# dvrp0/Monsoon

Hardware: AMD Instinct MI355X
Metric: env-steps/sec (whole node) at 65536 concurrent games; bit-exact vs CPU replay (higher is better)
Workload: dtype u8/i16 state, f64 draw+score

## Files before the change

monsoon_amd/csrc/abilities.inc:

```

MSB_HD MSB_INL PList sel_targets(int shape, P c, int pov, Tgt t) { return shape_targets(shape, c, pov, t, PK_NONE); }

MSB_HD MSB_INL bool sel_any(int shape, P c, int pov, Tgt t) { return shape_any(shape, c, pov, t); }

MSB_HD MSB_A_TILES PList empty_shape_tiles(int shape, P c, int pov) {
  PList raw = shape_tiles(shape, c, pov);
  PList out;
  out.clear();
  int m = raw.n();
  for (int i = 0; i < m; i++)
    if (at(raw.at(i)) == AT_NONE) out.push_raw(raw.get(i));
  return out;
}
MSB_HD MSB_A_TILES PList empty_within_front_line(int order) {
  PList out;
  out.clear();
  int fl = pl_front(order);
  if (order == 0) {
    for (int y = fl; y < 5; y++)
      for (int x = 0; x < 4; x++) {
        P p{x, y};
        if (at(p) == AT_NONE) out.push(p);
      }
  } else {
// ... 106 lines not shown
      const int who = at(l.at(i));
      if (who < 0 || who >= AT_PLAYER) {
        set_fault(who < 0 ? FAULT_PY_EXCEPTION : FAULT_UNSUPPORTED);
        break;
      }
      const int s = e_str(who);
      const int dealt = s - 3 < 0 ? s : 3;
      if (dealt < -128) set_fault(FAULT_UNSUPPORTED);
      cur = dealt & 0xff;
      call_damage(k, who, 3, true);
    } break;
    case EACH_DMG_RAND: {
      const int t = at(l.at(i));
      if (t < 0) {
        set_fault(FAULT_PY_EXCEPTION);
        break;
      }
      const int dmg = rng_randint(4, 6);
      call_damage(k, t, dmg, true);
    } break;
    case EACH_DESTROY: {
      const int t = at(l.at(i));
      if (t < 0 || t >= AT_PLAYER) {
        set_fault(t < 0 ? FAULT_PY_EXCEPTION : FAULT_UNSUPPORTED);
        break;
      }
      call_destroy(k, t, true);
    } break;
    case EACH_COMMAND:
      call_command(k, at(l.at(i)));
      break;
    case EACH_COMMAND_B203: {
      const int t = at(l.at(i));
      if (!need_unit(t)) break;
      if (e_confused(t)) deconfuse(t);
      if (fault()) break;
      call_command(k, t);
    } break;
    case EACH_U018: {
      Tgt t = mk_tgt(TK_ANY, TS_ENEMY);
      t = tgt_base(t);
      const PList l2 = get_targets(cp(), t, PK_NONE);
      call_damage(k, at(choice_point(l2)), 2, true);
    } break;
    case EACH_UE01: {
      const PList l2 = get_targets(arg, mk_tgt(TK_UNIT, TS_ENEMY), PK_NONE);
      if (l2.n() > 0) call_damage(k, at(choice_point(l2)), 1, true);
      else skip = true;
    } break;
    case EACH_U017: {
      const int me = cur;
      const int oi = l.get(i);
      int idx = oi;
      for (int q = 0; q < oi; q++)
        if (arg & (1 << q)) idx--;
      const CardInfo& ci = g_cards[hand_card(me, idx)];
      P pos{0, 0};
      bool has_pos = false;
      if (ci.tgt.has) {
        const PList l2 = get_targets(cp(), mk_tgt(ci.tgt), PK_NONE);
        if (l2.n() == 0) {
          set_fault(FAULT_PY_EXCEPTION);
          break;
        }
        pos = choice_point(l2);
        has_pos = true;
      }
      arg |= 1 << oi;
      call_player_play(k, me, idx, pos, has_pos);
    } break;
    default:
      set_fault(FAULT_UNSUPPORTED);
      break;
  }
  if (fault()) return;
  if (skip) {
    if (counts) n--;
    else i++;
  }
  m.sk_st(top - 1, (uint32_t)op | ((uint32_t)(arg & 0xff) << 8) | (counts ? (uint32_t)(n & 0xffff) << 16 : ((uint32_t)(i & 0xff) << 16) | ((uint32_t)(n & 0xff) << 24)));
  m.sk_st(top, mk_hdr(F_EACH, skip ? 0 : 1, e, cur));
}

enum : int {
  AFTER_U076 = 1,
  AFTER_U302,
  AFTER_B305,
};
MSB_HD MSB_INL void call_after(Wk& k, int op, int e, int t, int aux) {
  wk_push(k, (uint32_t)aux);
  wk_push(k, mk_hdr(F_AFTER, op, e, t));
}
MSB_HD MSB_INL void h_after(Wk& k, const uint32_t hdr) {
  const int top = k.sp - 1;
  const int op = hdr_st(hdr), t = hdr_b(hdr);
  const int aux = (int)m.sk_ld(top - 1);
  k.sp = top - 1;
  switch (op) {
// ... 34 lines not shown
    MSB_CARD_LOCALS                                                        \
    switch (0) {                                                           \
      default: __VA_ARGS__                                                 \
    }                                                                      \
  }
#define MSB_CARD_K(id, ...)                                                \
  MSB_HD MSB_A_RARE int ab_##id(int sp_, int deep_, int e, int pos_pk, bool src) { \
    Wk k{sp_, 0, deep_, 0};                                                \
    const int card = id;                                                   \
    MSB_CARD_LOCALS                                                        \
    switch (0) {                                                           \
      default: __VA_ARGS__                                                 \
    }                                                                      \
    return k.sp;                                                           \
  }
#define MSB_SPELL(id, ...)                                                 \
  MSB_HD MSB_A_CARD void sp_##id(int me, int pos_pk) {                     \
    const int card = id;                                                   \
    MSB_SPELL_LOCALS                                                       \
    switch (0) {                                                           \
      default: __VA_ARGS__                                                 \
    }                                                                      \
  }
#define MSB_SPELL_K(id, ...)                                               \
  MSB_HD MSB_A_RARE int sp_##id(int sp_, int deep_, int me, int pos_pk) {  \
    Wk k{sp_, 0, deep_, 0};                                                \
    const int card = id;                                                   \
    MSB_SPELL_LOCALS                                                       \
    switch (0) {                                                           \
      default: __VA_ARGS__                                                 \
    }                                                                      \
    return k.sp;                                                           \
  }
#include "ability_cases.inc"
#undef MSB_CARD
#undef MSB_CARD_K
#undef MSB_SPELL
#undef MSB_SPELL_K

MSB_HD MSB_INL void ability_entity_card(Wk& k, int card, int e, int pos_pk, bool src) {
  switch (card) {
#define MSB_CARD(id, ...) case id: ab_##id(e, pos_pk, src); break;
#define MSB_CARD_K(id, ...) case id: k.sp = ab_##id(k.sp, k.base - k.seg, e, pos_pk, src); break;
#define MSB_SPELL(id, ...)
#define MSB_SPELL_K(id, ...)
#include "ability_cases.inc"
#undef MSB_CARD
#undef MSB_CARD_K
#undef MSB_SPELL
#undef MSB_SPELL_K
    default:
      if (card_has_ability(card)) set_fault(FAULT_UNSUPPORTED);
      break;
  }
}
MSB_HD MSB_INL void ability_entity(Wk& k, int e, int pos_pk, bool src) {
  MSB_SCOPE(PS_ABILITY_ENTITY);
  const int card = e_card(e);
#if defined(__HIP_DEVICE_COMPILE__)
  int cv = card;
  asm volatile("" : "+v"(cv));
  for (unsigned long long todo = __ballot(1); todo;) {
    const int leader = __builtin_ctzll(todo);
    const int c0 = __builtin_amdgcn_readlane(card, leader), c1 = __builtin_amdgcn_readlane(cv, leader);
    const bool mine = card == c0;
    todo &= ~__ballot(mine);
    if (mine) {
// ... 47 lines not shown
```

monsoon_amd/csrc/ability_cases.inc:

```

MSB_CARD_K(C_B002, {
      l = get_targets(dpov, mk_tgt(TK_ANY, TS_ENEMY), PK_NONE);
      if (l.n() > 0) {
        l = sorted_head(l, 0, true, 1);
        call_damage(k, at(l.at(0)), 8, true);
      }
    } break;
)
MSB_CARD_K(C_B004, {
      Tgt t = mk_tgt(TK_ANY, TS_ENEMY);
      t = tgt_base(t);
      l = get_targets(dpov, t, PK_NONE);
      call_each(k, EACH_DMG_B004, e, l, l.n(), 4, 0);
    } break;
)
MSB_CARD(C_B005, {
      if (!REM_LISTS) {
        set_fault(FAULT_UNSUPPORTED);
        break;
      }
      l = sel_targets(SH_SURROUNDING, mypos, dpov, mk_tgt(TK_ANY, TS_FRIENDLY));
      int mine = m.ld8(E_REM + e);
      if (mine == REM_LOST) {
        set_fault(FAULT_CAP_REM);
// ... 125 lines not shown
      if (l.n() > 0) {
        l = sorted_head(l, 1, false, 1);
        call_destroy(k, at(l.at(0)), true);
      }
    } break;
)
MSB_CARD(C_B009, {
      l = get_targets(dpov, mk_tgt(TK_UNIT, TS_ENEMY), PK_NONE);
      if (l.n() > 0) {
        l = sorted_head(l, 0, true, 2);
        l = shuffle(l);
        for (int i = 0; i < l.n() && !fault(); i++) confuse(at(l.at(i)));
      }
    } break;
)
MSB_CARD(C_B104, {
      l = get_targets(dpov, mk_tgt(TK_UNIT, TS_ENEMY), PK_NONE);
      if (l.n() > 0) {
        l = sorted_head(l, 0, true, 1);
        freeze(at(l.at(0)));
      }
    } break;
)
MSB_CARD_K(C_B203, {
      l = sel_targets(SH_FRONT, mypos, me, mk_tgt(TK_UNIT, TS_FRIENDLY));
      call_each(k, EACH_COMMAND_B203, e, l, l.n(), 0, 0);
    } break;
)
MSB_CARD_K(C_B304,
      call_entity_damage(k, e, 3, false, true);
      break;
)
MSB_CARD(C_U007, {
      l = sel_targets(SH_SURROUNDING, mypos, me, mk_tgt(TK_UNIT, TS_ENEMY));
      if (l.n() > 0) {
        int t = at(choice_point(l));
        heal(t, 5);
        vitalize(t);
      }
    } break;
)
MSB_CARD_K(C_U017, {
      int hn = pl_hand_n(me);
      PList orig;
      orig.clear();
      for (int i = 0; i < hn; i++) {
        int c = hand_card(me, i);
        if (c < NUM_CARDS && g_cards[c].kind == KIND_SPELL && hand_cost(me, i) <= 8) orig.push_raw(i);
      }
      int nc = orig.n();
      if (nc == 0) break;
      orig = shuffle(orig);
      int remaining = 8;
      PList pick;
      pick.clear();
      for (int i = 0; i < nc; i++) {
        int cost = hand_cost(me, orig.get(i));
        if (cost <= remaining) {
          pick.push_raw(orig.get(i));
          remaining -= cost;
        }
      }
      call_each(k, EACH_U017, e, pick, pick.n(), 0, me);
    } break;
)
MSB_CARD_K(C_U018, {
      l = sel_targets(SH_SURROUNDING, mypos, dpov, mk_tgt(TK_UNIT, TS_ANY));
      int types = 0, cnt = 0;
      for (int i = 0; i < l.n(); i++) {
        int b = 1 << card_first_type(e_card(at(l.at(i))));
        if (!(types & b)) {
          types |= b;
          cnt++;
        }
      }
      call_each(k, EACH_U018, e, l, cnt, 0, 0);
    } break;
)
MSB_CARD(C_U021, {
      l = get_targets(dpov, mk_tgt(TK_UNIT, TS_FRIENDLY), p_pack(mypos));
      if (l.n() > 0) heal(at(choice_point(l)), 5);
    } break;
)
MSB_CARD_K(C_U026, {
      l = sel_targets(SH_BEHIND, mypos, dpov, mk_tgt(TK_ANY, TS_ENEMY));
      if (l.n() > 0) call_damage(k, at(l.at(0)), 6, true);
    } break;
)
MSB_CARD(C_U036,
      if (pl_hand_n(me) == 0) heal(at(mypos), 12);
      break;
)
MSB_CARD(C_U040, {
      if (src) {
        l = shape_tiles(SH_SURROUNDING, mypos, me);
        if (l.n() > 0) respawn(e, choice_point(l), 12);
      }
    } break;
)
MSB_CARD(C_U050,
      if (mypos.y == 4) gain_speed(e, 3);
      break;
)
MSB_CARD(C_U051, {
      if (!sel_any(SH_BORDERING, mypos, dpov, mk_tgt(TK_UNIT, TS_ANY)))
        gain_speed(e, 1);
      else
        heal(e, 2);
    } break;
)
MSB_CARD(C_U053, {
      if (!sel_any(SH_SURROUNDING, mypos, dpov, mk_tgt(TK_UNIT, TS_ANY))) {
        gain_speed(e, 2);
      } else {
        if (!sel_any(SH_BORDERING, mypos, dpov, mk_tgt(TK_UNIT, TS_ANY))) gain_speed(e, 1);
      }
    } break;
)
MSB_CARD(C_U055, {
      Tgt t = mk_tgt(TK_UNIT, TS_ENEMY);
      t = tgt_xstatus(t, 1 << ST_CONFUSED);
      l = sel_targets(SH_FRONT, mypos, dpov, t);
      for (int i = 0; i < l.n() && !fault(); i++) confuse(at(l.at(i)));
    } break;
)
MSB_CARD(C_U061, {
      confuse(e);
      l = get_targets(dpov, mk_tgt(TK_UNIT, TS_FRIENDLY), p_pack(mypos));
      if (l.n() > 0) confuse(at(choice_point(l)));
      gain_speed(e, 2);
    } break;
)
MSB_CARD(C_U071, {
      l = sel_targets(SH_BORDERING, mypos, me, mk_tgt(TK_UNIT, TS_ENEMY));
      PList nc;
      nc.clear();
      for (int i = 0; i < l.n(); i++)
        if (!e_confused(at(l.at(i)))) nc.push_raw(l.get(i));
      if (nc.n() > 0) {
        confuse(at(choice_point(nc)));
        l = shape_tiles(SH_FRONT, mypos, dpov);
        if (l.n() > 0 && at(l.at(0)) == AT_NONE) teleport(e, l.at(0));
      }
    } break;
)
MSB_CARD_K(C_U074, {
      l = sel_targets(SH_FRONT, mypos, me, mk_tgt(TK_UNIT, TS_ENEMY));
      if (l.n() > 0) call_force_attack(k, e, l.at(0));
    } break;
)
MSB_CARD_K(C_U076, {
      Tgt t = mk_tgt(TK_UNIT, TS_ANY);
      t = tgt_xtypes(t, 1 << UT_DRAGON);
      l = sel_targets(SH_SURROUNDING, mypos, dpov, t);
      if (l.n() > 0) {
        int target = at(choice_point(l));
        call_after(k, AFTER_U076, e, target, me);
        call_damage(k, target, 6, true);
      }
    } break;
)
MSB_CARD_K(C_U101, {
      P position = p_unpack(pos_pk);
      int t = at(position);
      if (p_is_base(position) || t < 0 || t >= AT_PLAYER || !e_is_unit(t) || !e_frozen(t)) break;
      Tgt tg = mk_tgt(TK_UNIT, TS_ENEMY);
      tg = tgt_status(tg, 1 << ST_FROZEN);
      l = sel_targets(SH_SURROUNDING, mypos, me, tg);
      call_each(k, EACH_DMG, e, l, l.n(), 8, 0);
    } break;
)
MSB_CARD(C_U103, {
      l = sel_targets(SH_BORDERING, mypos, dpov, mk_tgt(TK_UNIT, TS_ENEMY));
      for (int i = 0; i < l.n() && !fault(); i++) freeze(at(l.at(i)));
    } break;
)
MSB_CARD(C_U106, {
      if (sel_any(SH_BORDERING, mypos, dpov, mk_tgt(TK_STRUCTURE, TS_FRIENDLY)) || mypos.y == 4) heal(e, 7);
    } break;
)
MSB_CARD(C_U111, {
      for (int k = 0; k < 10 && !fault(); k++) {
        l = sel_targets(SH_SURROUNDING, mypos, me, mk_tgt(TK_UNIT, TS_FRIENDLY));
        if (l.n() > 0) heal(at(choice_point(l)), 1);
      }
    } break;
)
MSB_CARD(C_U117,
      freeze(e);
      break;
)
MSB_CARD(C_U206,
      player_deal_damage(me, 3);
      break;
)
MSB_CARD(C_U211, {
      l = shape_tiles(SH_FRONT, mypos, dpov);
      if (l.n() > 0 && at(l.at(0)) == AT_NONE) {
        int s = rng_randint(1, 3);
        spawn_token_unit(me, l.at(0), s, UT_SATYR);
      }
    } break;
)
MSB_CARD(C_U216,
      player_deal_damage(me, 2);
      break;
)
MSB_CARD(C_U217, {
      l = empty_shape_tiles(SH_ROW, P{0, 4}, dpov);
      if (l.n() > 0) spawn_token_unit(me, choice_point(l), 5, UT_SATYR);
    } break;
)
MSB_CARD_K(C_U302, {
      P position = p_unpack(pos_pk);
      int t = at(position);
      if (p_is_base(position) || t < 0 || t >= AT_PLAYER || !e_is_unit(t)) break;
      if (e_str(t) > e_str(e)) {
        call_after(k, AFTER_U302, e, t, p_tile(mypos));
        call_entity_damage(k, t, 7, false, true);
      }
    } break;
)
MSB_CARD(C_U305, {
      Tgt t = mk_tgt(TK_UNIT, TS_FRIENDLY);
      t = tgt_types(t, 1 << UT_CONSTRUCT);
      l = sel_targets(SH_BORDERING, mypos, dpov, t);
      if (l.n() > 0) {
        heal(at(choice_point(l)), 4);
        heal(e, 4);
      }
    } break;
)
MSB_CARD_K(C_U306, {
      l = get_targets(dpov, mk_tgt(TK_ANY, TS_FRIENDLY), p_pack(mypos));
      if (l.n() > 0) call_damage(k, at(choice_point(l)), 1, true);
    } break;
)
MSB_CARD(C_U310, {
      l = sel_targets(SH_BORDERING, mypos, dpov, mk_tgt(TK_UNIT, TS_ENEMY));
      int behind = -1, right = -1, left = -1, front = -1;
      for (int i = 0; i < l.n(); i++) {
        P t = l.at(i);
        if (behind < 0 && mypos.y + 1 == t.y) behind = i;
        if (right < 0 && mypos.x + 1 == t.x) right = i;
        if (left < 0 && mypos.x - 1 == t.x) left = i;
        if (front < 0 && mypos.y - 1 == t.y) front = i;
      }
      int target = -1;
      if (behind >= 0 && l.at(behind).y < 4 && at(P{l.at(behind).x, l.at(behind).y + 1}) == AT_NONE)
        target = behind;
      else if (left >= 0 && l.at(left).x > 0 && at(P{l.at(left).x - 1, l.at(left).y}) == AT_NONE)
        target = left;
      else if (right >= 0 && l.at(right).x < 3 && at(P{l.at(right).x + 1, l.at(right).y}) == AT_NONE)
        target = right;
      else if (front >= 0 && l.at(front).y > 0 && at(P{l.at(front).x, l.at(front).y - 1}) == AT_NONE)
        target = front;
      if (target < 0) {
        set_fault(FAULT_PY_EXCEPTION);
        break;
      }
      push_pull(at(l.at(target)), mypos, true);
    } break;
)
MSB_CARD(C_U313, {
      l = sel_targets(SH_SURROUNDING, mypos, dpov, mk_tgt(TK_UNIT, TS_FRIENDLY));
      if (l.n() > 0) heal(at(choice_point(l)), 5);
      heal(e, 5);
    } break;
)
MSB_CARD(C_U314, {
      l = sel_targets(SH_FRONT, mypos, dpov, mk_tgt(TK_UNIT, TS_FRIENDLY));
      if (l.n() > 0) push_pull(at(l.at(0)), mypos, true);
    } break;
)
MSB_CARD(C_U316, {
      l = sel_targets(SH_SURROUNDING, mypos, dpov, mk_tgt(TK_UNIT, TS_FRIENDLY));
      if (l.n() > 0) {
        l = shuffle(l);
        for (int i = 0; i < l.n() && i < 2 && !fault(); i++) vitalize(at(l.at(i)));
      }
      vitalize(e);
    } break;
)
MSB_CARD(C_U320, {
      l = sel_targets(SH_SURROUNDING, mypos, me, mk_tgt(TK_UNIT, TS_FRIENDLY));
      if (l.n() > 0) heal(at(choice_point(l)), 4);
    } break;
)
MSB_CARD_K(C_U401, {
      l = sel_targets(SH_BORDERING, mypos, dpov, mk_tgt(TK_UNIT, TS_ANY));
      call_each(k, EACH_DMG_POISON, e, l, l.n(), 5, 0);
    } break;
)
MSB_CARD(C_U403, {
      Tgt t = mk_tgt(TK_UNIT, TS_ANY);
      t = tgt_status(t, 1 << ST_POISONED);
      l = sel_targets(SH_SURROUNDING, mypos, dpov, t);
      for (int i = 0; i < l.n() && !fault(); i++) {
        PList tiles;
        tiles = empty_shape_tiles(SH_BORDERING, l.at(i), dpov);
        tiles = shuffle(tiles);
        for (int k = 0; k < tiles.n() && k < 4 && !fault(); k++) spawn_token_unit(me, tiles.at(k), 1, UT_TOAD);
      }
    } break;
)
MSB_CARD_K(C_U405, {
      l = sel_targets(SH_BORDERING, mypos, dpov, mk_tgt(TK_UNIT, TS_ANY));
      call_each(k, EACH_DMG_HEAL, e, l, l.n(), 3, 0);
    } break;
)
MSB_CARD(C_U406, {
      l = empty_shape_tiles(SH_BORDERING, mypos, dpov);
      if (l.n() > 0) {
        P tile = choice_point(l);
        spawn_token_unit(opponent_of(me), tile, 1, UT_RAVEN);
      }
    } break;
)
MSB_CARD(C_U411, {
// ... 24 lines not shown
        l.clear();
        for (int i = 0; i < side.n(); i++)
          if (e_str(at(side.at(i))) == mn) l.push_raw(side.get(i));
        if (l.n() > 0) call_destroy(k, at(choice_point(l)), true);
      }
    } break;
)
MSB_CARD(C_UA05, {
      l = empty_shape_tiles(SH_SIDE, mypos, dpov);
      for (int i = 0; i < l.n() && !fault(); i++) spawn_token_unit(me, l.at(i), 4, UT_ANCIENT);
    } break;
)
MSB_CARD(C_UA07, {
      switch (rng_randint(0, 5)) {
        case 0: freeze(e); break;
        case 1: poison(e); break;
        case 2: vitalize(e); break;
        case 3: confuse(e); break;
        case 4: disable(e); break;
      }
    } break;
)
MSB_CARD(C_UA20, {
      if (!sel_any(SH_FRONT, mypos, me, mk_tgt(TK_UNIT, TS_ENEMY))) {
        const int cand[4] = {C_B005, C_B006, C_B203, C_B305};
        int c = cand[rng_randint(0, 4)];
        if (ctx() == 0) push_new_instance(me, false, c, 0, CF_SINGLE_USE | CF_XBASE, g_cards[c].strength);
      }
    } break;
)
MSB_CARD(C_UD01, {
      Tgt t = mk_tgt(TK_UNIT, TS_FRIENDLY);
      t = tgt_types(t, 1 << UT_DRAGON);
      l = get_targets(me, t, PK_NONE);
      if (l.n() > 0) heal(at(choice_point(l)), 7);
    } break;
)
MSB_CARD_K(C_UD02, {
      Tgt t = mk_tgt(TK_UNIT, TS_ANY);
      t = tgt_xtypes(t, 1 << UT_DRAGON);
      l = sel_targets(SH_FRONT, mypos, dpov, t);
      call_each(k, EACH_DMG, e, l, l.n(), 4, 0);
    } break;
)
MSB_CARD(C_UD31, {
      P position = p_unpack(pos_pk);
      int t = at(position);
      if (p_is_base(position) || t < 0 || t >= AT_PLAYER || !e_is_unit(t)) break;
      Tgt tg = mk_tgt(TK_UNIT, TS_FRIENDLY);
      tg = tgt_types(tg, 1 << UT_DRAGON);
      l = sel_targets(SH_SURROUNDING, mypos, me, tg);
      if (l.n() > 0) heal(at(choice_point(l)), 2);
      heal(e, 2);
    } break;
)
MSB_CARD_K(C_UE01, {
      int n = e_dmg(e);
      if (n > 0xffff) set_fault(FAULT_UNSUPPORTED);
      l.clear();
      if (n > 0 && n <= 0xffff) call_each(k, EACH_UE01, e, l, n, me, 0);
    } break;
)
MSB_CARD(C_UE03, {
      l = empty_shape_tiles(SH_BORDERING, mypos, dpov);
      if (l.n() > 0) {
        P tile = choice_point(l);
        spawn_token_unit(me, tile, e_str(e), UT_ELDER);
      }
    } break;
)
MSB_CARD(C_UE04, {
      l = get_targets(me, mk_tgt(TK_UNIT, TS_ENEMY), PK_NONE);
      int cnt = 0;
      for (int i = 0; i < l.n(); i++)
        if (e_str(at(l.at(i))) > e_str(e)) cnt++;
      heal(e, cnt * 4);
    } break;
)
MSB_CARD(C_UE05, {
      Tgt t = mk_tgt(TK_UNIT, TS_FRIENDLY);
      t = tgt_limit(t, e_str(e) - 1);
      l = get_targets(me, t, p_pack(mypos));
      for (int i = 0; i < l.n() && i < 4; i++) e_set_str(at(l.at(i)), e_str(e));
    } break;
)
// ... 54 lines not shown
MSB_CARD(C_UP03, {
      l = get_targets(dpov, mk_tgt(TK_UNIT, TS_FRIENDLY), PK_NONE);
      int types = 0;
      for (int i = 0; i < l.n(); i++) types |= card_types(e_card(at(l.at(i))));
      int amount = 3 * __builtin_popcount(types);
      l = sel_targets(SH_SURROUNDING, mypos, dpov, mk_tgt(TK_UNIT, TS_ENEMY));
      for (int i = 0; i < l.n(); i++) {
        int t = at(l.at(i));
        int s = e_str(t) - amount;
        e_set_str(t, s > 1 ? s : 1);
      }
    } break;
)

MSB_SPELL_K(C_S001,
      call_damage(k, at(position), 9, true);
      break;
)
MSB_SPELL_K(C_S003, {
      l = get_targets(dpov, mk_tgt(TK_ANY, TS_ENEMY), PK_NONE);
      call_each(k, EACH_DMG_RAND, 0xff, l, l.n(), 0, 0);
    } break;
)
MSB_SPELL(C_S004, {
      l = empty_within_front_line(me);
      if (l.n() > 0) {
        l = shuffle(l);
        int amount = rng_randint(6, 7);
        for (int i = 0; i < l.n() && i < amount && !fault(); i++) spawn_token_unit(me, l.at(i), 1, UT_TOAD);
      }
    } break;
)
MSB_SPELL(C_S007, {
      int t = at(position);
      heal(t, 7);
      if (!fault()) vitalize(t);
    } break;
)
MSB_SPELL(C_S012, {
      l = empty_within_front_line(me);
      if (l.n() > 0) spawn_token_unit(me, choice_point(l), 5, UT_KNIGHT);
    } break;
)
MSB_SPELL_K(C_S013, {
      PList picked;
      picked.clear();
      for (int ut = 0; ut < 16; ut++) {
        Tgt t = mk_tgt(TK_UNIT, TS_ANY);
        t = tgt_types(t, 1 << ut);
        l = get_targets(dpov, t, PK_NONE);
        PList units;
        units.clear();
        for (int i = 0; i < l.n(); i++)
          if (!picked.has(l.at(i))) units.push_raw(l.get(i));
        if (units.n() > 0) picked.push(choice_point(units));
      }
      call_each(k, EACH_DMG, 0xff, picked, picked.n(), 6, 0);
    } break;
)
MSB_SPELL(C_S021, {
      confuse(at(position));
      if (fault()) break;
      Tgt t = mk_tgt(TK_UNIT, TS_FRIENDLY);
      t = tgt_types(t, 1 << UT_FELINE);
      l = get_targets(dpov, t, PK_NONE);
      if (l.n() > 0) {
        int mn = 32767;
        for (int i = 0; i < l.n(); i++) {
          int s = e_str(at(l.at(i)));
          if (s < mn) mn = s;
        }
        PList w;
        w.clear();
        for (int i = 0; i < l.n(); i++)
// ... 14 lines not shown
    } break;
)
MSB_SPELL_K(C_S104, {
      int t = at(position);
      if (!need_unit(t)) break;
      if (e_frozen(t))
        call_entity_damage(k, t, 12, false, true);
      else
        freeze(t);
    } break;
)
MSB_SPELL(C_S105,
      heal(at(position), 15);
      break;
)
MSB_SPELL_K(C_S203, {
      l = s203_targets(dpov);
      call_each(k, EACH_DMG, 0xff, l, l.n(), 6, 0);
    } break;
)
MSB_SPELL_K(C_S302, {
      Tgt t = mk_tgt(TK_ANY, TS_ENEMY);
      t = tgt_base(t);
      l = get_targets(dpov, t, PK_NONE);
      l = shuffle(l);
      call_each(k, EACH_DMG, 0xff, l, l.n() < 4 ? l.n() : 4, 4, 0);
    } break;
)
MSB_SPELL(C_S403, {
      Tgt t = mk_tgt(TK_UNIT, TS_FRIENDLY);
      t = tgt_status(t, 1 << ST_POISONED);
      l = get_targets(dpov, t, PK_NONE);
      for (int i = 0; i < l.n() && !fault(); i++) {
        int u = at(l.at(i));
        heal(u, 5);
        if (!fault()) vitalize(u);
      }
    } break;
)
```

monsoon_amd/csrc/rules.h:

```cpp
#pragma once
#include "mt19937.h"
#include "pyset.h"
#include "state.h"

#if defined(MSB_FAULT_TRACE) && !defined(__HIPCC__)
#include <execinfo.h>
#include <stdio.h>
static inline void msb_fault_trace(int code) {
  void* bt[24];
  int n = backtrace(bt, 24);
  fprintf(stderr, "set_fault(%d)\n", code);
  backtrace_symbols_fd(bt, n, 2);
}
#endif

#if defined(MSB_COUNT_FRAMES) && !defined(__HIPCC__)
#define MSB_COUNT_EVENT(i_) msb_frame_count[i_]++
#define MSB_COUNT_MAX(i_, v_) (msb_frame_count[i_] = (v_) > msb_frame_count[i_] ? (v_) : msb_frame_count[i_])
static long long msb_frame_count[64];
#else
#define MSB_COUNT_EVENT(i_)
#define MSB_COUNT_MAX(i_, v_)
#endif

// ... 1404 lines not shown
#else
    return shape_targets_full(shape, c, pov, t, exclude_pk);
#endif
  }
  MSB_HD MSB_INL PList shape_targets_full(int shape, P c, int pov, Tgt t, int exclude_pk) {
    PList all = get_targets_full(pov, t, exclude_pk);
    PList out;
    out.clear();
    bool base_rule = shape_base_rule(shape);
    int m = all.n();
    for (int i = 0; i < m; i++) {
      P p = all.at(i);
      if (in_shape(shape, c, pov, p) || (base_rule && p_is_base(p) && tg_base(t))) out.push_raw(all.get(i));
    }
    if (shape == SH_FRONT || shape == SH_BEHIND) sort_by_y(out, (shape == SH_FRONT) ? (pov == local()) : (pov == remote()));
    return out;
  }
  MSB_HD MSB_INL bool shape_any(const int shape, const P c, const int pov, const Tgt t) {
#if MSB_TARGET_SCAN
    MSB_SCOPE(PS_GET_TARGETS);
    if (get_targets_hit(pov, t, shape_mask(shape, c, pov)) != 0) return true;
    const int bases = target_bases(t);
    if (!bases) return false;
    const bool asc = (pov == local());
    return shape_base_rule(shape) || ((bases & 1) && in_shape(shape, c, pov, base_point(true, asc))) ||
           ((bases & 2) && in_shape(shape, c, pov, base_point(false, asc)));
#else
    return shape_targets_full(shape, c, pov, t, PK_NONE).n() > 0;
#endif
  }

  MSB_HD MSB_INL int choice_index(int n) { return rng_randint(0, n); }
  MSB_HD MSB_INL P choice_point(PList l) { return l.at(choice_index(l.n())); }
  MSB_HD MSB_A_SHUFFLE PList shuffle(PList l) {
    for (int i = l.n() - 1; i >= 1; i--) {
      int j = (int)rng_interval((uint32_t)i);
      int tmp = l.get(i);
      l.set(i, l.get(j));
      l.set(j, tmp);
    }
    return l;
  }
  MSB_HD MSB_A_SHUFFLE PList sorted_head(PList l, int key_mode, bool rev, int k) {
    int b0 = -1, b1 = -1, k0 = 0, k1 = 0;
    double r0 = 0.0, r1 = 0.0;
    int m = l.n();
    for (int i = 0; i < m; i++) {
      P p = l.at(i);
      int kv = key_mode == 0 ? p.y : e_str(at(p));
      double rv = rng_random_sample();
      bool lt0 = b0 < 0 || (rev ? (kv > k0 || (kv == k0 && rv > r0)) : (kv < k0 || (kv == k0 && rv < r0)));
      if (lt0) {
        b1 = b0; k1 = k0; r1 = r0;
        b0 = i; k0 = kv; r0 = rv;
      } else {
        bool lt1 = b1 < 0 || (rev ? (kv > k1 || (kv == k1 && rv > r1)) : (kv < k1 || (kv == k1 && rv < r1)));
        if (lt1) {
          b1 = i; k1 = kv; r1 = rv;
        }
      }
    }
    PList out;
    out.clear();
    if (b0 >= 0 && k >= 1) out.push_raw(l.get(b0));
    if (b1 >= 0 && k >= 2) out.push_raw(l.get(b1));
    return out;
// ... 278 lines not shown
#else
  MSB_HD MSB_INL void call_destroy(Wk& k, int e, bool src) {
    const int sv = ctx_enter(e);
    if (fault()) return;
    wk_push_ctx(k, sv);
    if (e_is_unit(e)) {
      board_set(e_pos(e), -1);
      m.st8g(eg(e), EO_PATHN, 0);
      e_set_dmg(e, e_str(e));
      if (e_card_trigger(e) == TR_ON_DEATH) {
        push_trigger(e, src);
        if (fault()) return;
        if (!m.ld8(H_RESOLVING)) {
          wk_push(k, mk_hdr(F_DESTROY_TAIL, 0, 0, 0));
          call_pop_trigger(k);
          return;
        }
      }
      recalc_front_after_destroy();
    } else {
      e_set_dmg(e, e_str(e));
      board_set(e_pos(e), -1);
      recalc_front_after_destroy();
    }
  }
#endif
  MSB_HD MSB_INL bool need_unit(int e) {
    if (e < 0 || e >= AT_PLAYER || !e_is_unit(e)) {
      set_fault(FAULT_PY_EXCEPTION);
      return false;
    }
    return true;
  }
  MSB_HD MSB_INL void freeze(int e) {
    if (need_unit(e)) e_st_add(e, ST_FROZEN);
  }
  MSB_HD MSB_INL void poison(int e) {
    if (!need_unit(e)) return;
    if (e_st(e, ST_VITALIZED) > 0) e_st_remove(e, ST_VITALIZED);
    e_st_add(e, ST_POISONED);
  }
  MSB_HD MSB_INL void vitalize(int e) {
    if (!need_unit(e)) return;
    if (e_st(e, ST_POISONED) > 0) e_st_remove(e, ST_POISONED);
    e_st_add(e, ST_VITALIZED);
  }
  MSB_HD MSB_INL void confuse(int e) {
    if (need_unit(e)) e_st_add(e, ST_CONFUSED);
  }
  MSB_HD MSB_INL void deconfuse(int e) {
    if (need_unit(e)) e_st_remove(e, ST_CONFUSED);
  }
  MSB_HD MSB_INL void disable(int e) {
    if (need_unit(e) && e_has_ability(e)) e_st_add(e, ST_DISABLED);
  }

  MSB_HD MSB_INL void set_path(int e, bool on_play) {
    const int sv = ctx_enter(e);
    set_path_impl(e, on_play);
    ctx_leave(sv);
  }
#if MSB_WE_IMG && MSB_WIDE_PATH
  MSB_HD MSB_A_SETPATH void set_path_impl(int e, bool on_play) { set_path_known(e, on_play, m.ld32g(eg(e), 0)); }
  MSB_HD MSB_A_SETPATH void set_path_known(int e, bool on_play, const uint32_t ge) {
#else
  MSB_HD MSB_A_SETPATH void set_path_impl(int e, bool on_play) {
#endif
    MSB_SCOPE(PS_SET_PATH);
#if MSB_WIDE_PATH
    static_assert(EO_CARD == 0 && EO_FLAGS == 1 && EO_POS == 2 && EO_MOV == 3, "word 0 of an entity");
#if !MSB_WE_IMG
    const uint32_t ge = m.ld32g(eg(e), 0);
#endif
    P position = tile_p((int)(ge >> 16) & 0xff);
    int confused_cached = e_st(e, ST_CONFUSED);
    const int owner = (int)(ge >> 8) & EF_OWNER;
    const bool ff = ((ge >> 8) & EF_FF) != 0;
    const bool is_local = owner == local();
    const int steps = on_play ? (int)(ge >> 24) : 1;
    uint32_t packed = 0;
    int n = 0, nd = 0;
    uint32_t seen = 0;
    for (int k = 0; k < steps; k++) {
      P dest{position.x, position.y + (is_local ? -1 : 1)};
      if (confused_cached > 0) {
        int dx;
        if (position.x == 0)
          dx = 1;
// ... 490 lines not shown
#undef MV_WAIT
#undef MV_CALLED
  }
#endif

  MSB_HD MSB_INL void call_unit_play(Wk& k, int e, P position) {
#if MSB_WE_IMG && MSB_WIDE_PATH
    const uint32_t w0 = ((m.ld32g(eg(e), 0) | ((uint32_t)EF_RESOLVING_PLAY << 8)) & ~0xff0000u) | ((uint32_t)(p_tile(position) & 0xff) << 16);
    const int kind = e_kind(e);
    m.st32g(eg(e), 0, w0);
    board_put(p_tile(position), e);
    set_path_known(e, true, w0);
    if (fault()) return;
    if (kind_card_trigger(kind) == TR_ON_PLAY) {
#else
    e_set_flag(e, EF_RESOLVING_PLAY, true);
    board_set(position, e);
    set_path(e, true);
    if (fault()) return;
    if (e_card_trigger(e) == TR_ON_PLAY) {
#endif
      call_move_later(k, e, MV_PLAYED);
      call_run_ability(k, e, -1, PK_NONE, true);
    } else {
      call_move(k, e, MV_PLAYED);
    }
  }
  MSB_HD MSB_INL void call_structure_play(Wk& k, int e, P position) {
    board_set(position, e);
    if (e_card_trigger(e) == TR_ON_PLAY) call_run_ability(k, e, -1, PK_NONE, true);
  }
  MSB_HD MSB_INL bool e_resolving_play(int e) const { return (e_flags(e) & EF_RESOLVING_PLAY) != 0; }
  MSB_HD MSB_INL void gain_speed(int e, int amount) {
    int mv = e_mov(e);
    m.st8g(eg(e), EO_MOV, mv + amount);
    set_path(e, e_resolving_play(e));
    m.st8g(eg(e), EO_MOV, mv);
  }
  MSB_HD MSB_INL void call_command(Wk& k, int e) {
    if (!need_unit(e)) return;
    const int sv = ctx_enter(e);
    if (fault()) return;
    wk_push_ctx(k, sv);
    const bool ff = e_ff(e);
    e_set_flag(e, EF_FF, true);
    set_path(e, false);
    if (fault()) return;
    wk_push(k, mk_hdr(F_CMD_TAIL, 0, e, ff ? 1 : 0));
    call_move(k, e);
  }
  MSB_HD MSB_INL void convert(int e) {
    int o = e_owner(e);
    int no = opponent_of(o);
    e_set_flag(e, EF_OWNER, no != 0);
    set_path(e, e_resolving_play(e));
  }
  MSB_HD MSB_INL void teleport(int e, P dest) {
    const int sv = ctx_enter(e);
    teleport_impl(e, dest);
    ctx_leave(sv);
  }
  MSB_HD MSB_A_MISC void teleport_impl(int e, P dest) {
    if (at(dest) == AT_NONE) {
      board_set(e_pos(e), -1);
      board_set(dest, e);
      int o = e_owner(e);
      if (pl_front(o) > dest.y) set_pl_front(o, dest.y > 1 ? dest.y : 1);
      set_path(e, e_resolving_play(e));
    }
  }
// ... 610 lines not shown
      }
    }
    PList playable;
    playable.clear();
    for (int i = 0; i < 4; i++) {
      bool any = false;
      for (int a = 16 * i; a <= 16 * i + 15 && !any; a++) any = (lm[0] >> a) & 1;
      for (int a = 21 * i + 64; a <= 21 * i + 84 && !any; a++) any = a < 128 ? ((lm[1] >> (a - 64)) & 1) : ((lm[2] >> (a - 128)) & 1);
      if (any) playable.push_raw(i);
    }
    if (playable.n() > 0) {
      bool exact = false;
      int min_cost = 1 << 20;
      for (int k = 0; k < playable.n(); k++) {
        int c = hand_cost(lo, playable.get(k));
        if (c == mana) exact = true;
        if (c < min_cost) min_cost = c;
      }
      int want = exact ? mana : min_cost;
      PList pick;
      pick.clear();
      for (int k = 0; k < playable.n(); k++)
        if (hand_cost(lo, playable.get(k)) == want) pick.push_raw(k);
      int index = playable.get(pick.get(choice_index(pick.n())));
      int card = hand_card(lo, index);
      const CardInfo& ci = g_cards[card];
      PList enemies = get_targets(cp(), mk_tgt(TK_UNIT, TS_ENEMY), PK_NONE);
      PList bbe;
      bbe.clear();
      for (int k = 0; k < enemies.n(); k++)
        if (enemies.at(k).y == 4) bbe.push_raw(enemies.get(k));
      if (ci.kind == KIND_SPELL) {
        if (!ci.tgt.has) return 64 + 21 * index;
        PList t = get_targets(cp(), mk_tgt(ci.tgt), PK_NONE);
        if (t.n() == 0) {
          set_fault(FAULT_PY_EXCEPTION);
          return 155;
        }
        P p = choice_point(t);
        return p_valid(p) ? 65 + 21 * index + (4 - p.y) * 4 + p.x : 155;
      } else if (ci.kind == KIND_UNIT && bbe.n() > 0) {
        PList cand;
        cand.clear();
        for (int k = 0; k < bbe.n(); k++) {
          P en = bbe.at(k);
          if (en.x > 0 && at(P{en.x - 1, en.y}) == AT_NONE)
            cand.push(P{en.x - 1, en.y});
          else if (en.x < 3 && at(P{en.x + 1, en.y}) == AT_NONE)
            cand.push(P{en.x + 1, en.y});
        }
        if (cand.n() > 0) {
          P p = choice_point(cand);
          return p.y >= 1 ? 16 * index + (4 - p.y) * 4 + p.x : 155;
        }
      } else {
        int fl = pl_front(lo);
        PList cand;
        cand.clear();
        for (int x = 0; x < 4; x++)
          if (at(P{x, fl}) == AT_NONE) cand.push(P{x, fl});
        for (int k = 0; k < enemies.n(); k++) {
          P en = enemies.at(k);
          if (en.x > 0 && en.y >= fl && at(P{en.x - 1, en.y}) == AT_NONE)
            cand.push(P{en.x - 1, en.y});
          else if (en.x < 3 && en.y >= fl && at(P{en.x + 1, en.y}) == AT_NONE)
            cand.push(P{en.x + 1, en.y});
          else if (en.y < 4 && en.y + 1 >= fl && at(P{en.x, en.y + 1}) == AT_NONE)
            cand.push(P{en.x, en.y + 1});
        }
        if (cand.n() > 0) {
          P p = choice_point(cand);
          return p.y >= 1 ? 16 * index + (4 - p.y) * 4 + p.x : 155;
// ... 69 lines not shown
```

monsoon_amd/csrc/state.h:

```cpp
#pragma once
#include "msb_base.h"
#include "lds_layout.h"

namespace msb {

#if defined(MSB_CAP_ENT)
constexpr int NUM_ENT = MSB_CAP_ENT;
#elif defined(MSB_EXT) && MSB_EXT == 2
constexpr int NUM_ENT = 254;
#elif defined(MSB_EXT) && MSB_EXT
constexpr int NUM_ENT = 64;
#else
constexpr int NUM_ENT = 24;
#endif
constexpr int HAND_CAP = 5;
constexpr int DECK_SIZE = 12;
#if defined(MSB_EXT) && MSB_EXT
#if MSB_EXT == 2
constexpr int DECK_CAP = 48;
#else
constexpr int DECK_CAP = 28;
#endif
#if defined(MSB_CAP_REM)
constexpr int REM_LISTS = MSB_CAP_REM, WORLD_CAP = MSB_CAP_WORLD;
// ... 90 lines not shown
constexpr int DRAW_HINT_LDS = WK_OVF_LDS + 8;
#ifndef MSB_COOP_DRAW
#define MSB_COOP_DRAW 1
#endif
#ifndef MSB_COOP_LEGAL
#define MSB_COOP_LEGAL 1
#endif
#ifndef MSB_TARGET_SCAN
#define MSB_TARGET_SCAN 1
#endif
#ifndef MSB_WIDE_LISTS
#define MSB_WIDE_LISTS 1
#endif
#ifndef MSB_WIDE_PATH
#define MSB_WIDE_PATH 1
#endif
#ifndef MSB_WIDE_ENT
#define MSB_WIDE_ENT 1
#endif
#ifndef MSB_WIDE_ENT_HDR
#define MSB_WIDE_ENT_HDR 0
#endif
#ifndef MSB_WIDE_ENT_IMG
#define MSB_WIDE_ENT_IMG MSB_WIDE_ENT
#endif
#if defined(MSB_EXT) && MSB_EXT
#define MSB_WE_HDR 0
#define MSB_WE_IMG 0
#else
#define MSB_WE_HDR MSB_WIDE_ENT_HDR
#define MSB_WE_IMG MSB_WIDE_ENT_IMG
#endif
#define MSB_WE_ANY (MSB_WE_HDR || MSB_WE_IMG)
constexpr int LDS_RECORDS = WK_OVF_LDS + 16;
constexpr int SK_CAP = 640;
constexpr int SK_MARGIN = 32;
constexpr int SK_NEED = 12;
constexpr int CF_SINGLE_USE = 1, CF_FF = 2, CF_STR = 4, CF_ALIAS = 8;
constexpr int CF_XBASE = 16, CF_SPELL = 32;

constexpr int OFF_ENT = (OFF_PL + 2 * PL_SIZE + 15) & ~15;
constexpr int ENT_SIZE = 16;
constexpr int EO_CARD = 0;
constexpr int EO_FLAGS = 1;
constexpr int EO_POS = 2;
constexpr int EO_MOV = 3;
constexpr int EO_ST = 4;
constexpr int EO_MOVEID = 9;
constexpr int EO_STR = 10;
constexpr int EO_DMG = 12;
constexpr int EO_PATHN = 14;
constexpr int EO_KIND = 15;
constexpr int EK_UNIT = 1, EK_ABILITY = 2;
constexpr int E_PATH = OFF_ENT + ENT_SIZE * NUM_ENT;
constexpr int E_REM = E_PATH + 4 * NUM_ENT;
constexpr int E_HOME = E_REM + (REM_LISTS ? NUM_ENT : 0);
constexpr int OFF_REM = (E_HOME + (REM_LISTS ? NUM_ENT : 0) + 3) & ~3;
constexpr int OFF_WORLD = (OFF_REM + REM_LISTS * REM_LIST_BYTES + 3) & ~3;
constexpr int USED_WORDS = (NUM_ENT + 31) / 32;
constexpr bool TRIG_WIDE = NUM_ENT > 128;
constexpr int TRIG_SLOT = TRIG_WIDE ? 0xff : 0x7f;
constexpr int OFF_X = OFF_WORLD + WORLD_CAP * WORLD_BYTES;
constexpr int X_CTX = OFF_X, X_RNGBLK = OFF_X + 2, X_SEED = OFF_X + 4, X_USED_HI = OFF_X + 8;
constexpr int X_TRIGSRC = X_USED_HI + 4 * (USED_WORDS - 1);
constexpr int X_BYTES = REM_LISTS ? (X_TRIGSRC - OFF_X) + (TRIG_WIDE ? 4 : 0) : 0;
constexpr int STATE_BYTES = (OFF_X + X_BYTES + 15) & ~15;
// ... 296 lines not shown
```

Baseline: 2.210 billion.

## Pick random ability targets from bitmasks instead of materialized point lists

```diff
diff --git a/monsoon_amd/csrc/abilities.inc b/monsoon_amd/csrc/abilities.inc
--- a/monsoon_amd/csrc/abilities.inc
+++ b/monsoon_amd/csrc/abilities.inc
@@ -162,20 +162,19 @@
       break;
     case EACH_COMMAND_B203: {
       const int t = at(l.at(i));
-      if (!need_unit(t)) break;
-      if (e_confused(t)) deconfuse(t);
+      if (!deconfuse_if_confused(t)) break;
       if (fault()) break;
       call_command(k, t);
     } break;
     case EACH_U018: {
       Tgt t = mk_tgt(TK_ANY, TS_ENEMY);
       t = tgt_base(t);
-      const PList l2 = get_targets(cp(), t, PK_NONE);
-      call_damage(k, at(choice_point(l2)), 2, true);
+      const Pick q = targets_pick(cp(), t, PK_NONE);
+      call_damage(k, at(choice_tile(q)), 2, true);
     } break;
     case EACH_UE01: {
-      const PList l2 = get_targets(arg, mk_tgt(TK_UNIT, TS_ENEMY), PK_NONE);
-      if (l2.n() > 0) call_damage(k, at(choice_point(l2)), 1, true);
+      const Pick q = targets_pick(arg, mk_tgt(TK_UNIT, TS_ENEMY), PK_NONE);
+      if (q.n() > 0) call_damage(k, at(choice_tile(q)), 1, true);
       else skip = true;
     } break;
     case EACH_U017: {
@@ -188,12 +187,12 @@
       P pos{0, 0};
       bool has_pos = false;
       if (ci.tgt.has) {
-        const PList l2 = get_targets(cp(), mk_tgt(ci.tgt), PK_NONE);
-        if (l2.n() == 0) {
+        const Pick q = targets_pick(cp(), mk_tgt(ci.tgt), PK_NONE);
+        if (q.n() == 0) {
           set_fault(FAULT_PY_EXCEPTION);
           break;
         }
-        pos = choice_point(l2);
+        pos = choice_tile(q);
         has_pos = true;
       }
       arg |= 1 << oi;
@@ -294,7 +293,16 @@
     }                                                                      \
     return k.sp;                                                           \
   }
+#if MSB_AB_ST
+#define MSB_HEAL_VITALIZE(who, amount) heal_vitalize(who, amount, false)
+#define MSB_HEAL_VITALIZE_CHECKED(who, amount) heal_vitalize(who, amount, true)
+#else
+#define MSB_HEAL_VITALIZE(who, amount) { int t = who; heal(t, amount); vitalize(t); }
+#define MSB_HEAL_VITALIZE_CHECKED(who, amount) { int t = who; heal(t, amount); if (!fault()) vitalize(t); }
+#endif
 #include "ability_cases.inc"
+#undef MSB_HEAL_VITALIZE
+#undef MSB_HEAL_VITALIZE_CHECKED
 #undef MSB_CARD
 #undef MSB_CARD_K
 #undef MSB_SPELL
diff --git a/monsoon_amd/csrc/ability_cases.inc b/monsoon_amd/csrc/ability_cases.inc
--- a/monsoon_amd/csrc/ability_cases.inc
+++ b/monsoon_amd/csrc/ability_cases.inc
@@ -181,12 +181,8 @@
       break;
 )
 MSB_CARD(C_U007, {
-      l = sel_targets(SH_SURROUNDING, mypos, me, mk_tgt(TK_UNIT, TS_ENEMY));
-      if (l.n() > 0) {
-        int t = at(choice_point(l));
-        heal(t, 5);
-        vitalize(t);
-      }
+      const Pick q = shape_pick(SH_SURROUNDING, mypos, me, mk_tgt(TK_UNIT, TS_ENEMY));
+      if (q.n() > 0) MSB_HEAL_VITALIZE(at(choice_tile(q)), 5);
     } break;
 )
 MSB_CARD_K(C_U017, {
@@ -227,8 +223,8 @@
     } break;
 )
 MSB_CARD(C_U021, {
-      l = get_targets(dpov, mk_tgt(TK_UNIT, TS_FRIENDLY), p_pack(mypos));
-      if (l.n() > 0) heal(at(choice_point(l)), 5);
+      const Pick q = targets_pick(dpov, mk_tgt(TK_UNIT, TS_FRIENDLY), p_pack(mypos));
+      if (q.n() > 0) heal(at(choice_tile(q)), 5);
     } break;
 )
 MSB_CARD_K(C_U026, {
@@ -275,8 +271,8 @@
 )
 MSB_CARD(C_U061, {
       confuse(e);
-      l = get_targets(dpov, mk_tgt(TK_UNIT, TS_FRIENDLY), p_pack(mypos));
-      if (l.n() > 0) confuse(at(choice_point(l)));
+      const Pick q = targets_pick(dpov, mk_tgt(TK_UNIT, TS_FRIENDLY), p_pack(mypos));
+      if (q.n() > 0) confuse(at(choice_tile(q)));
       gain_speed(e, 2);
     } break;
 )
@@ -301,9 +297,9 @@
 MSB_CARD_K(C_U076, {
       Tgt t = mk_tgt(TK_UNIT, TS_ANY);
       t = tgt_xtypes(t, 1 << UT_DRAGON);
-      l = sel_targets(SH_SURROUNDING, mypos, dpov, t);
-      if (l.n() > 0) {
-        int target = at(choice_point(l));
+      const Pick q = shape_pick(SH_SURROUNDING, mypos, dpov, t);
+      if (q.n() > 0) {
+        int target = at(choice_tile(q));
         call_after(k, AFTER_U076, e, target, me);
         call_damage(k, target, 6, true);
       }
@@ -330,8 +326,8 @@
 )
 MSB_CARD(C_U111, {
       for (int k = 0; k < 10 && !fault(); k++) {
-        l = sel_targets(SH_SURROUNDING, mypos, me, mk_tgt(TK_UNIT, TS_FRIENDLY));
-        if (l.n() > 0) heal(at(choice_point(l)), 1);
+        const Pick q = shape_pick(SH_SURROUNDING, mypos, me, mk_tgt(TK_UNIT, TS_FRIENDLY));
+        if (q.n() > 0) heal(at(choice_tile(q)), 1);
       }
     } break;
 )
@@ -373,16 +369,16 @@
 MSB_CARD(C_U305, {
       Tgt t = mk_tgt(TK_UNIT, TS_FRIENDLY);
       t = tgt_types(t, 1 << UT_CONSTRUCT);
-      l = sel_targets(SH_BORDERING, mypos, dpov, t);
-      if (l.n() > 0) {
-        heal(at(choice_point(l)), 4);
+      const Pick q = shape_pick(SH_BORDERING, mypos, dpov, t);
+      if (q.n() > 0) {
+        heal(at(choice_tile(q)), 4);
         heal(e, 4);
       }
     } break;
 )
 MSB_CARD_K(C_U306, {
-      l = get_targets(dpov, mk_tgt(TK_ANY, TS_FRIENDLY), p_pack(mypos));
-      if (l.n() > 0) call_damage(k, at(choice_point(l)), 1, true);
+      const Pick q = targets_pick(dpov, mk_tgt(TK_ANY, TS_FRIENDLY), p_pack(mypos));
+      if (q.n() > 0) call_damage(k, at(choice_tile(q)), 1, true);
     } break;
 )
 MSB_CARD(C_U310, {
@@ -412,8 +408,8 @@
     } break;
 )
 MSB_CARD(C_U313, {
-      l = sel_targets(SH_SURROUNDING, mypos, dpov, mk_tgt(TK_UNIT, TS_FRIENDLY));
-      if (l.n() > 0) heal(at(choice_point(l)), 5);
+      const Pick q = shape_pick(SH_SURROUNDING, mypos, dpov, mk_tgt(TK_UNIT, TS_FRIENDLY));
+      if (q.n() > 0) heal(at(choice_tile(q)), 5);
       heal(e, 5);
     } break;
 )
@@ -432,8 +428,8 @@
     } break;
 )
 MSB_CARD(C_U320, {
-      l = sel_targets(SH_SURROUNDING, mypos, me, mk_tgt(TK_UNIT, TS_FRIENDLY));
-      if (l.n() > 0) heal(at(choice_point(l)), 4);
+      const Pick q = shape_pick(SH_SURROUNDING, mypos, me, mk_tgt(TK_UNIT, TS_FRIENDLY));
+      if (q.n() > 0) heal(at(choice_tile(q)), 4);
     } break;
 )
 MSB_CARD_K(C_U401, {
@@ -524,8 +520,8 @@
 MSB_CARD(C_UD01, {
       Tgt t = mk_tgt(TK_UNIT, TS_FRIENDLY);
       t = tgt_types(t, 1 << UT_DRAGON);
-      l = get_targets(me, t, PK_NONE);
-      if (l.n() > 0) heal(at(choice_point(l)), 7);
+      const Pick q = targets_pick(me, t, PK_NONE);
+      if (q.n() > 0) heal(at(choice_tile(q)), 7);
     } break;
 )
 MSB_CARD_K(C_UD02, {
@@ -541,8 +537,8 @@
       if (p_is_base(position) || t < 0 || t >= AT_PLAYER || !e_is_unit(t)) break;
       Tgt tg = mk_tgt(TK_UNIT, TS_FRIENDLY);
       tg = tgt_types(tg, 1 << UT_DRAGON);
-      l = sel_targets(SH_SURROUNDING, mypos, me, tg);
-      if (l.n() > 0) heal(at(choice_point(l)), 2);
+      const Pick q = shape_pick(SH_SURROUNDING, mypos, me, tg);
+      if (q.n() > 0) heal(at(choice_tile(q)), 2);
       heal(e, 2);
     } break;
 )
@@ -663,14 +659,12 @@
     } break;
 )
 MSB_SPELL(C_S007, {
-      int t = at(position);
-      heal(t, 7);
-      if (!fault()) vitalize(t);
+      MSB_HEAL_VITALIZE_CHECKED(at(position), 7);
     } break;
 )
 MSB_SPELL(C_S012, {
-      l = empty_within_front_line(me);
-      if (l.n() > 0) spawn_token_unit(me, choice_point(l), 5, UT_KNIGHT);
+      const Pick q = empty_front_pick(me);
+      if (q.n() > 0) spawn_token_unit(me, choice_tile(q), 5, UT_KNIGHT);
     } break;
 )
 MSB_SPELL_K(C_S013, {
@@ -751,9 +745,7 @@
       t = tgt_status(t, 1 << ST_POISONED);
       l = get_targets(dpov, t, PK_NONE);
       for (int i = 0; i < l.n() && !fault(); i++) {
-        int u = at(l.at(i));
-        heal(u, 5);
-        if (!fault()) vitalize(u);
-      }
-    } break;
-)
+        MSB_HEAL_VITALIZE_CHECKED(at(l.at(i)), 5);
+      }
+    } break;
+)
diff --git a/monsoon_amd/csrc/rules.h b/monsoon_amd/csrc/rules.h
--- a/monsoon_amd/csrc/rules.h
+++ b/monsoon_amd/csrc/rules.h
@@ -1460,6 +1460,54 @@
 
   MSB_HD MSB_INL int choice_index(int n) { return rng_randint(0, n); }
   MSB_HD MSB_INL P choice_point(PList l) { return l.at(choice_index(l.n())); }
+#if MSB_AB_PICK
+  struct Pick {
+    uint32_t hit;
+    int bases;
+    bool asc;
+    MSB_HD MSB_INL int n() const { return __builtin_popcount(hit) + (bases & 1) + ((bases >> 1) & 1); }
+  };
+  MSB_HD MSB_INL P choice_tile(uint32_t hit, const int bases, const bool asc) {
+    const int nt = __builtin_popcount(hit);
+    int r = choice_index(nt + (bases & 1) + ((bases >> 1) & 1));
+    if ((unsigned)r < (unsigned)nt) {
+      if (!asc) r = nt - 1 - r;
+      for (; r > 0; r--) hit &= hit - 1;
+      return tile_p(__builtin_ctz(hit));
+    }
+    return base_point((bases & 1) && r == nt, asc);
+  }
+  MSB_HD MSB_INL P choice_tile(const Pick& q) { return choice_tile(q.hit, q.bases, q.asc); }
+  MSB_HD MSB_A_TARGETS Pick targets_pick(int pov, Tgt t, int exclude_pk) {
+    MSB_SCOPE(PS_GET_TARGETS);
+    const bool asc = (pov == local());
+    uint32_t tiles = 0xFFFFFu;
+    int bases = target_bases(t);
+    exclude_point(exclude_pk, asc, tiles, bases);
+    return Pick{get_targets_hit(pov, t, tiles), bases, asc};
+  }
+  MSB_HD MSB_A_SHAPE Pick shape_pick(int shape, P c, int pov, Tgt t) {
+    MSB_SCOPE(PS_GET_TARGETS);
+    const bool asc = (pov == local());
+    int bases = target_bases(t);
+    if (bases && !shape_base_rule(shape))
+      bases &= (in_shape(shape, c, pov, base_point(true, asc)) ? 1 : 0) | (in_shape(shape, c, pov, base_point(false, asc)) ? 2 : 0);
+    return Pick{get_targets_hit(pov, t, shape_mask(shape, c, pov)), bases, asc};
+  }
+  MSB_HD MSB_INL Pick empty_front_pick(int order) {
+    const int fl = pl_front(order);
+    return Pick{~occ_mask() & (order == 0 ? 0xFFFFFu & ~rows_below(fl) : rows_below(fl + 1)), 0, order == 0};
+  }
+#else
+  struct Pick {
+    PList l;
+    MSB_HD MSB_INL int n() const { return l.n(); }
+  };
+  MSB_HD MSB_INL P choice_tile(const Pick& q) { return choice_point(q.l); }
+  MSB_HD MSB_INL Pick targets_pick(int pov, Tgt t, int exclude_pk) { return Pick{get_targets(pov, t, exclude_pk)}; }
+  MSB_HD MSB_INL Pick shape_pick(int shape, P c, int pov, Tgt t) { return Pick{shape_targets(shape, c, pov, t, PK_NONE)}; }
+  MSB_HD MSB_INL Pick empty_front_pick(int order) { return Pick{empty_within_front_line(order)}; }
+#endif
   MSB_HD MSB_A_SHUFFLE PList shuffle(PList l) {
     for (int i = l.n() - 1; i >= 1; i--) {
       int j = (int)rng_interval((uint32_t)i);
@@ -1804,6 +1852,76 @@
     }
     return true;
   }
+#if MSB_AB_ST
+  MSB_HD MSB_INL bool ei_need_unit(int e, EImg& g) {
+    if (e < 0 || e >= AT_PLAYER) {
+      set_fault(FAULT_PY_EXCEPTION);
+      return false;
+    }
+    g = ei_load(e);
+    if (!(ei_kind(g, e) & EK_UNIT)) {
+      set_fault(FAULT_PY_EXCEPTION);
+      return false;
+    }
+    return true;
+  }
+  MSB_HD MSB_INL void ei_st_add(int e, EImg& g, int s) {
+    const int c = ei_st(g, e, s);
+    if (c >= 255) {
+      set_fault(FAULT_STATUS_SAT);
+      return;
+    }
+    m.st8g(eg(e), EO_ST + s, c + 1);
+    ei_put8(g, EO_ST + s, c + 1);
+  }
+  MSB_HD MSB_INL void ei_st_remove(int e, EImg& g, int s) {
+    const int c = ei_st(g, e, s);
+    if (c == 0) {
+      set_fault(FAULT_PY_EXCEPTION);
+      return;
+    }
+    m.st8g(eg(e), EO_ST + s, c - 1);
+    ei_put8(g, EO_ST + s, c - 1);
+  }
+  MSB_HD MSB_INL void ei_poison(int e, EImg& g) {
+    if (ei_st(g, e, ST_VITALIZED) > 0) ei_st_remove(e, g, ST_VITALIZED);
+    ei_st_add(e, g, ST_POISONED);
+  }
+  MSB_HD MSB_INL void ei_vitalize(int e, EImg& g) {
+    if (ei_st(g, e, ST_POISONED) > 0) ei_st_remove(e, g, ST_POISONED);
+    ei_st_add(e, g, ST_VITALIZED);
+  }
+  MSB_HD MSB_INL void freeze(int e) {
+    EImg g;
+    if (ei_need_unit(e, g)) ei_st_add(e, g, ST_FROZEN);
+  }
+  MSB_HD MSB_INL void poison(int e) {
+    EImg g;
+    if (ei_need_unit(e, g)) ei_poison(e, g);
+  }
+  MSB_HD MSB_INL void vitalize(int e) {
+    EImg g;
+    if (ei_need_unit(e, g)) ei_vitalize(e, g);
+  }
+  MSB_HD MSB_INL void confuse(int e) {
+    EImg g;
+    if (ei_need_unit(e, g)) ei_st_add(e, g, ST_CONFUSED);
+  }
+  MSB_HD MSB_INL void deconfuse(int e) {
+    EImg g;
+    if (ei_need_unit(e, g)) ei_st_remove(e, g, ST_CONFUSED);
+  }
+  MSB_HD MSB_INL void disable(int e) {
+    EImg g;
+    if (ei_need_unit(e, g) && (ei_kind(g, e) & EK_ABILITY)) ei_st_add(e, g, ST_DISABLED);
+  }
+  MSB_HD MSB_INL bool deconfuse_if_confused(int e) {
+    EImg g;
+    if (!ei_need_unit(e, g)) return false;
+    if (ei_st(g, e, ST_CONFUSED) > 0) ei_st_remove(e, g, ST_CONFUSED);
+    return true;
+  }
+#else
   MSB_HD MSB_INL void freeze(int e) {
     if (need_unit(e)) e_st_add(e, ST_FROZEN);
   }
@@ -1826,6 +1944,31 @@
   MSB_HD MSB_INL void disable(int e) {
     if (need_unit(e) && e_has_ability(e)) e_st_add(e, ST_DISABLED);
   }
+  MSB_HD MSB_INL bool deconfuse_if_confused(int e) {
+    if (!need_unit(e)) return false;
+    if (e_confused(e)) deconfuse(e);
+    return true;
+  }
+#endif
+#if MSB_AB_ST
+  MSB_HD MSB_INL void heal_vitalize(int who, int amount, bool checked) {
+    if (who >= 0 && who < AT_PLAYER) {
+      EImg g = ei_load(who);
+      const int s = ei_str(g, who) + amount;
+      e_set_str(who, s);
+      ei_put_str(g, s);
+      if (checked && fault()) return;
+      if (!(ei_kind(g, who) & EK_UNIT)) {
+        set_fault(FAULT_PY_EXCEPTION);
+        return;
+      }
+      ei_vitalize(who, g);
+      return;
+    }
+    heal(who, amount);
+    if (!checked || !fault()) vitalize(who);
+  }
+#endif
 
   MSB_HD MSB_INL void set_path(int e, bool on_play) {
     const int sv = ctx_enter(e);
@@ -2382,10 +2525,15 @@
   }
   MSB_HD MSB_INL bool e_resolving_play(int e) const { return (e_flags(e) & EF_RESOLVING_PLAY) != 0; }
   MSB_HD MSB_INL void gain_speed(int e, int amount) {
+#if MSB_AB_SPEED
+    const uint32_t w0 = m.ld32g(eg(e), 0);
+    set_path_known(e, ((w0 >> 8) & EF_RESOLVING_PLAY) != 0, (w0 & 0x00ffffffu) | ((((w0 >> 24) + (uint32_t)amount) & 0xffu) << 24));
+#else
     int mv = e_mov(e);
     m.st8g(eg(e), EO_MOV, mv + amount);
     set_path(e, e_resolving_play(e));
     m.st8g(eg(e), EO_MOV, mv);
+#endif
   }
   MSB_HD MSB_INL void call_command(Wk& k, int e) {
     if (!need_unit(e)) return;
@@ -3062,12 +3210,12 @@
         if (enemies.at(k).y == 4) bbe.push_raw(enemies.get(k));
       if (ci.kind == KIND_SPELL) {
         if (!ci.tgt.has) return 64 + 21 * index;
-        PList t = get_targets(cp(), mk_tgt(ci.tgt), PK_NONE);
+        const Pick t = targets_pick(cp(), mk_tgt(ci.tgt), PK_NONE);
         if (t.n() == 0) {
           set_fault(FAULT_PY_EXCEPTION);
           return 155;
         }
-        P p = choice_point(t);
+        P p = choice_tile(t);
         return p_valid(p) ? 65 + 21 * index + (4 - p.y) * 4 + p.x : 155;
       } else if (ci.kind == KIND_UNIT && bbe.n() > 0) {
         PList cand;
diff --git a/monsoon_amd/csrc/state.h b/monsoon_amd/csrc/state.h
--- a/monsoon_amd/csrc/state.h
+++ b/monsoon_amd/csrc/state.h
@@ -146,6 +146,24 @@
 #define MSB_WE_IMG MSB_WIDE_ENT_IMG
 #endif
 #define MSB_WE_ANY (MSB_WE_HDR || MSB_WE_IMG)
+#ifndef MSB_WIDE_AB_ST
+#define MSB_WIDE_AB_ST 0
+#endif
+#ifndef MSB_WIDE_AB_SPEED
+#define MSB_WIDE_AB_SPEED 0
+#endif
+#ifndef MSB_WIDE_AB_PICK
+#define MSB_WIDE_AB_PICK 1
+#endif
+#if defined(MSB_EXT) && MSB_EXT
+#define MSB_AB_ST 0
+#define MSB_AB_SPEED 0
+#define MSB_AB_PICK 0
+#else
+#define MSB_AB_ST (MSB_WIDE_AB_ST && MSB_WE_IMG)
+#define MSB_AB_SPEED (MSB_WIDE_AB_SPEED && MSB_WE_IMG && MSB_WIDE_PATH)
+#define MSB_AB_PICK (MSB_WIDE_AB_PICK && MSB_TARGET_SCAN)
+#endif
 constexpr int LDS_RECORDS = WK_OVF_LDS + 16;
 constexpr int SK_CAP = 640;
 constexpr int SK_MARGIN = 32;
```

Result: faster. 2.246 billion, median of 6 (+1.6%).
